# pytorch/audio

Measured on AMD Instinct MI355X. Metric: audio-sec/sec MelSpectrogram (b=256, 16kHz, n_fft=400, n_mels=80), higher is better.
Workload: dtype f32; 1 GPU; MelSpectrogram n_fft=400 hop=160 n_mels=80, batch=256 x 10 s @16 kHz fp32 per GPU (BASELINE configs[1]); per_gpu_batch=256

## Files before the change

audio_amd/csrc/melspec400.h:

```cpp
#pragma once
#include <cstdint>
#include <cstring>
#include <type_traits>
#include "hd.h"
#include "stft_generic.h"

namespace aamd {
namespace m400 {

constexpr int kN = 400;
constexpr int kPad = 200;
constexpr int kFramesPerWave = 6;
#ifndef AAMD_M400_WAVES
#define AAMD_M400_WAVES 12
#define AAMD_M400_MINWAVES 3
#endif
constexpr int kWavesPerBlock = AAMD_M400_WAVES;
constexpr int kTOff[20] = {0, 260, 520, 652, 784, 916, 1444, 1576, 128, 388,
                           2104, 2232, 2364, 1708, 1840, 1048, 1180, 1312, 1972, 2492};
constexpr int kTBufDwords = 2492 + 128;
constexpr int kTRow = 44;
constexpr int kTPair = 20 * kTRow;
constexpr int kLdsDwordsPerWave = 3 * kTPair;
constexpr int kPK = 208;
// ... 485 lines not shown
  const float m = sqrt(m2);
  if (power == 1.0f) return m;
  return pow(m, power);
}

AAMD_HD void phase_b2_spec(const LaneConst& c, const float (&zr)[20], const float (&zi)[20],
                           const float (&xr)[10], const float (&xi)[10], float power, int phase, float* lds) {
  if (!c.active) return;
  float* Ra = lds + phase + kSpecBins * 2 * c.p + c.col;
  float* Rb = Ra + kSpecBins;
#pragma unroll
  for (int u = 0; u < 10; ++u) {
    const float cr = xr[9 - u], ci = xi[9 - u];
    const float ar = zr[u] + cr, ai = zi[u] - ci;
    const float br = zr[u] - cr, bi = zi[u] + ci;
    Ra[20 * u] = spec_pow(ar * ar + ai * ai, power);
    Rb[20 * u] = spec_pow(br * br + bi * bi, power);
  }
  if (c.col == 0) {
    const float ar = zr[10] + zr[10], bi = zi[10] + zi[10];
    Ra[200] = spec_pow(ar * ar, power);
    Rb[200] = spec_pow(bi * bi, power);
  }
}

AAMD_HD void phase_b2_spec_complex(const LaneConst& c, const float (&zr)[20], const float (&zi)[20],
                                   const float (&xr)[10], const float (&xi)[10], int half, int phase, float* lds) {
  if (!c.active) return;
  const int fa = 2 * c.p - 3 * half, fb = fa + 1;
  const bool wa = fa >= 0 && fa < 3, wb = fb >= 0 && fb < 3;
  float* Ra = lds + phase + 2 * kSpecBins * fa + 2 * c.col;
  float* Rb = lds + phase + 2 * kSpecBins * fb + 2 * c.col;
#pragma unroll
  for (int u = 0; u < 10; ++u) {
    const float cr = xr[9 - u], ci = xi[9 - u];
    if (wa) { Ra[40 * u] = zr[u] + cr; Ra[40 * u + 1] = zi[u] - ci; }
    if (wb) { Rb[40 * u] = zi[u] + ci; Rb[40 * u + 1] = cr - zr[u]; }
  }
  if (c.col == 0) {
    if (wa) { Ra[400] = zr[10] + zr[10]; Ra[401] = 0.0f; }
    if (wb) { Rb[400] = zi[10] + zi[10]; Rb[401] = 0.0f; }
  }
}

AAMD_HD void store_spec(int lane, const float* lds, float* out, int64_t a0, int n_floats) {
  const int phase = (int)(a0 & 3);
  float* base = out + (a0 - phase);
  const int n_pieces = (phase + n_floats + 3) >> 2;
  for (int j = lane; j < n_pieces; j += 64) {
    const int i0 = 4 * j;
    if (i0 >= phase && i0 + 4 <= phase + n_floats) {
      *reinterpret_cast<F4*>(base + i0) = *reinterpret_cast<const F4*>(lds + i0);
    } else {
      for (int e = 0; e < 4; ++e)
        if (i0 + e >= phase && i0 + e < phase + n_floats) base[i0 + e] = lds[i0 + e];
    }
  }
}

#ifndef AAMD_M400_SPEC_FULL
#define AAMD_M400_SPEC_FULL 1
#endif
AAMD_HD void store_spec_full(int lane, const float* lds, float* out, int64_t a0) {
  constexpr int kN = kFramesPerWave * kSpecBins;
  const int phase = (int)(a0 & 3);
  float* base = out + (a0 - phase);
  const int n_pieces = (phase + kN + 3) >> 2;
  F4 v[5];
#pragma unroll
  for (int u = 0; u < 5; ++u) {
    const int j = lane + 64 * u;
    if (u < 4 || j < n_pieces) v[u] = *reinterpret_cast<const F4*>(lds + 4 * j);
  }
#pragma unroll
  for (int u = 0; u < 5; ++u) {
    const int j = lane + 64 * u, i0 = 4 * j;
    const bool full = i0 >= phase && i0 + 4 <= phase + kN;
    if ((u < 4 || j < n_pieces) && full) *reinterpret_cast<F4*>(base + i0) = v[u];
  }
  if (lane == 0 && phase != 0) {
    const float e[4] = {v[0].x, v[0].y, v[0].z, v[0].w};
#pragma unroll
    for (int k = 1; k < 4; ++k)
      if (k >= phase) base[k] = e[k];
  }
  const int jl = n_pieces - 1, il = 4 * jl;
  if (lane + 256 == jl && il + 4 > phase + kN) {
    const float e[4] = {v[4].x, v[4].y, v[4].z, v[4].w};
#pragma unroll
    for (int k = 0; k < 3; ++k)
      if (il + k < phase + kN) base[il + k] = e[k];
  }
}

AAMD_HD float fast_log10(float x) {
#if defined(__HIP_DEVICE_COMPILE__)
  return __log2f(x) * 0.30102999566398120f;
#else
  return log10(x);
#endif
}
AAMD_HD float epi_plog(float x) {
  const float kE = 2.718281828459045f;
#if defined(__HIP_DEVICE_COMPILE__)
  const float lg = __log2f(x) * 0.69314718055994531f;
#else
  const float lg = log(x);
#endif
  const float t = x > kE ? lg : x;
  return t <= kE ? t / kE : t;
}
AAMD_HD float epi_db(float x, const Epi400& e) {
  return e.multiplier * fast_log10(fmax(x, e.amin)) - e.db_sub;
}

AAMD_HD void phase_b2_pad(int lane, float* lds) {
  constexpr int kTail = kPK - 201;
  if (lane < 3 * kTail) {
    const int p = lane / kTail, j = lane - p * kTail;
    *reinterpret_cast<F2*>(lds + kPPair * p + 2 * (201 + j)) = F2{0.0f, 0.0f};
  }
}

template <int NC>
AAMD_HD void mel_chunks(const float* wt, const float* P, float& sa, float& sb) {
  F4 w[NC], q0[NC], q1[NC];
#pragma unroll
  for (int k = 0; k < NC; ++k) {
    w[k] = *reinterpret_cast<const F4*>(wt + 4 * k);
    q0[k] = *reinterpret_cast<const F4*>(P + 8 * k);
    q1[k] = *reinterpret_cast<const F4*>(P + 8 * k + 4);
  }
#pragma unroll
  for (int k = 0; k < NC; ++k) {
    sa += w[k].x * q0[k].x;
    sb += w[k].x * q0[k].y;
    sa += w[k].y * q0[k].z;
    sb += w[k].y * q0[k].w;
    sa += w[k].z * q1[k].x;
    sb += w[k].z * q1[k].y;
    sa += w[k].w * q1[k].z;
    sb += w[k].w * q1[k].w;
  }
}

template <int NR>
struct MelRegs {
  int nc[NR];
  int pm[NR];
  AAMD_HD int poff(int r) const { return pm[r] & 0xffff; }
  AAMD_HD int mel(int r) const { return pm[r] >> 16; }
};

template <int NR>
AAMD_HD void mel_regs_load(const LaneConst& c, const MelTab& mt, MelRegs<NR>& h) {
#pragma unroll
  for (int r = 0; r < NR; ++r) {
    const bool on = r < mt.n_rounds;
    const int row = r * kMelSlots + c.pi;
#if defined(__HIP_DEVICE_COMPILE__)
    h.nc[r] = on ? __builtin_amdgcn_readfirstlane(mt.rc[r]) : 0;
#else
    h.nc[r] = on ? mt.rc[r] : 0;
#endif
    const int poff = on ? 2 * mt.lo2[row] : 0;
    const int mel = on ? mt.row_mel[row] : -1;
    h.pm[r] = (int)(((unsigned)mel << 16) | (unsigned)poff);
  }
}

AAMD_HD constexpr int sig_chunks(int sig, int r) { return (sig >> (4 * r)) & 15; }
constexpr int kSigHtk80 = 0x4221, kSigSlaney80 = 0x4211;

template <int NR = kMelMaxRounds, int SIG = 0, bool FENCED = false>
AAMD_HD void phase_c(const LaneConst& c, const MelTab& mt, const float* lds,
                     float (&acc_a)[NR], float (&acc_b)[NR], const MelRegs<NR>* h = nullptr) {
  const float* Pp = lds + kPPair * c.p;
  const float* wt0 = mt.w + c.pi * mt.ws;
#pragma unroll
  for (int r = 0; r < NR; ++r) {
    float sa = 0.0f, sb = 0.0f;
#if defined(__HIP_DEVICE_COMPILE__)
    if (FENCED && SIG != 0 && r > 0 && (r & 1) == 0) __builtin_amdgcn_sched_barrier(0);
#endif
    if (SIG != 0 || r < mt.n_rounds) {
      const float* wt = wt0 + r * kMelSlots * mt.ws;
      const float* P = Pp + (h ? h->poff(r) : 2 * mt.lo2[r * kMelSlots + c.pi]);
      const int nc = SIG != 0 ? sig_chunks(SIG, r) : (h ? h->nc[r] : mt.rc[r]);
      switch (nc) {
        case 1: mel_chunks<1>(wt, P, sa, sb); break;
        case 2: mel_chunks<2>(wt, P, sa, sb); break;
        case 3: mel_chunks<3>(wt, P, sa, sb); break;
        case 4: mel_chunks<4>(wt, P, sa, sb); break;
        default:
          for (int k = 0; k < nc; ++k) mel_chunks<1>(wt + 4 * k, P + 8 * k, sa, sb);
      }
    }
    acc_a[r] = sa;
    acc_b[r] = sb;
  }
}

template <int OFF>
AAMD_HD void store_f32_saddr(float v, char* base, unsigned voff) {
#if defined(__HIP_DEVICE_COMPILE__)
  asm volatile("global_store_dword %0, %1, %2 offset:%3" : : "v"(voff), "v"(v), "s"(base), "i"(OFF) : "memory");
#else
  *reinterpret_cast<float*>(base + (size_t)voff + OFF) = v;
#endif
}

template <int NR = kMelMaxRounds, int SIG = 0>
AAMD_HD void store_direct(const LaneConst& c, const MelTab& mt, const float (&acc_a)[NR],
                          const float (&acc_b)[NR], float* out_row, int64_t t0, int n_frames,
                          const MelRegs<NR>* h = nullptr) {
  const int left = (int)(n_frames - t0);
  const bool va = c.active && 2 * c.p < left, vb = c.active && 2 * c.p + 1 < left;
  float* out_tile = out_row + t0 * (int64_t)mt.n_mels;
  const unsigned oa = 2u * (unsigned)c.p * (unsigned)mt.n_mels;
  if (SIG != 0) {
    constexpr unsigned nm = kMelSlots * NR;
    char* const ob = reinterpret_cast<char*>(out_row + t0 * (int64_t)nm);
    unsigned bo[NR];
#pragma unroll
    for (int r = 0; r < NR; ++r) bo[r] = 4u * (2u * (unsigned)c.p * nm + (unsigned)h->mel(r));
    if (left >= kFramesPerWave) {
      if (c.active) {
#pragma unroll
        for (int r = 0; r < NR; ++r) store_f32_saddr<0>(acc_a[r], ob, bo[r]);
#pragma unroll
        for (int r = 0; r < NR; ++r) store_f32_saddr<4 * (int)nm>(acc_b[r], ob, bo[r]);
      }
      return;
    }
    if (va) {
#pragma unroll
      for (int r = 0; r < NR; ++r) store_f32_saddr<0>(acc_a[r], ob, bo[r]);
    }
    if (vb) {
#pragma unroll
      for (int r = 0; r < NR; ++r) store_f32_saddr<4 * (int)nm>(acc_b[r], ob, bo[r]);
    }
    return;
  }
#pragma unroll
  for (int r = 0; r < NR; ++r) {
    if (r < mt.n_rounds) {
      const int m = h ? h->mel(r) : mt.row_mel[r * kMelSlots + c.pi];
      if (m >= 0) {
        if (va) out_tile[oa + (unsigned)m] = acc_a[r];
        if (vb) out_tile[oa + (unsigned)mt.n_mels + (unsigned)m] = acc_b[r];
      }
    }
  }
}

template <int NR = kMelMaxRounds>
AAMD_HD void store_stage(const LaneConst& c, const MelTab& mt, const float (&acc_a)[NR],
                         const float (&acc_b)[NR], float* lds, const MelRegs<NR>* h = nullptr) {
  if (!c.active) return;
  float* oa = lds + 2 * c.p * mt.n_mels;
#pragma unroll
  for (int r = 0; r < NR; ++r) {
    if (r < mt.n_rounds) {
      const int m = h ? h->mel(r) : mt.row_mel[r * kMelSlots + c.pi];
      if (m >= 0) {
        oa[m] = acc_a[r];
        oa[mt.n_mels + m] = acc_b[r];
      }
    }
  }
}

AAMD_HD void store_wide(int lane, const MelTab& mt, const float* lds, float* out_row, int64_t t0,
                        int n_frames) {
  const int64_t left = n_frames - t0;
  const int n_valid = left < kFramesPerWave ? (int)left : kFramesPerWave;
  const int pieces = n_valid * mt.n_mels / 4;
  float* dst = out_row + t0 * (int64_t)mt.n_mels;
  for (int j = lane; j < pieces; j += 64)
    *reinterpret_cast<F4*>(dst + 4 * j) = *reinterpret_cast<const F4*>(lds + 4 * j);
}

#if defined(__HIPCC__)
__device__ __forceinline__ float vmax_raw(float x, float y) {
  float r;
  asm("v_max_f32 %0, %1, %2" : "=v"(r) : "v"(x), "v"(y));
  return r;
}
__device__ __forceinline__ float vmin_raw(float x, float y) {
  float r;
  asm("v_min_f32 %0, %1, %2" : "=v"(r) : "v"(x), "v"(y));
  return r;
}
__device__ __forceinline__ float vmax3_raw(float x, float y, float z) {
  float r;
  asm("v_max3_f32 %0, %1, %2, %3" : "=v"(r) : "v"(x), "v"(y), "v"(z));
  return r;
}
__device__ __forceinline__ float vmin3_raw(float x, float y, float z) {
  float r;
  asm("v_min3_f32 %0, %1, %2, %3" : "=v"(r) : "v"(x), "v"(y), "v"(z));
  return r;
}
__device__ __forceinline__ void wave_lds_fence() {
  asm volatile("" ::: "memory");
}

__device__ __forceinline__ void exchange_partner(float (&qr)[10], float (&qi)[10], unsigned long long self_mask) {
  unsigned long long saved;
  asm volatile(
      "s_mov_b64 %[sv], exec\n\t"
      "s_andn2_b64 exec, exec, %[m]\n\t"
      "s_nop 4\n\t"
      "v_mov_b32_dpp %0, %0 quad_perm:[1,0,3,2] row_mask:0xf bank_mask:0xf\n\t"
      "v_mov_b32_dpp %1, %1 quad_perm:[1,0,3,2] row_mask:0xf bank_mask:0xf\n\t"
      "v_mov_b32_dpp %2, %2 quad_perm:[1,0,3,2] row_mask:0xf bank_mask:0xf\n\t"
      "v_mov_b32_dpp %3, %3 quad_perm:[1,0,3,2] row_mask:0xf bank_mask:0xf\n\t"
      "v_mov_b32_dpp %4, %4 quad_perm:[1,0,3,2] row_mask:0xf bank_mask:0xf\n\t"
      "v_mov_b32_dpp %5, %5 quad_perm:[1,0,3,2] row_mask:0xf bank_mask:0xf\n\t"
      "v_mov_b32_dpp %6, %6 quad_perm:[1,0,3,2] row_mask:0xf bank_mask:0xf\n\t"
      "v_mov_b32_dpp %7, %7 quad_perm:[1,0,3,2] row_mask:0xf bank_mask:0xf\n\t"
      "v_mov_b32_dpp %8, %8 quad_perm:[1,0,3,2] row_mask:0xf bank_mask:0xf\n\t"
      "v_mov_b32_dpp %9, %9 quad_perm:[1,0,3,2] row_mask:0xf bank_mask:0xf\n\t"
      "v_mov_b32_dpp %10, %10 quad_perm:[1,0,3,2] row_mask:0xf bank_mask:0xf\n\t"
      "v_mov_b32_dpp %11, %11 quad_perm:[1,0,3,2] row_mask:0xf bank_mask:0xf\n\t"
      "v_mov_b32_dpp %12, %12 quad_perm:[1,0,3,2] row_mask:0xf bank_mask:0xf\n\t"
      "v_mov_b32_dpp %13, %13 quad_perm:[1,0,3,2] row_mask:0xf bank_mask:0xf\n\t"
      "v_mov_b32_dpp %14, %14 quad_perm:[1,0,3,2] row_mask:0xf bank_mask:0xf\n\t"
      "v_mov_b32_dpp %15, %15 quad_perm:[1,0,3,2] row_mask:0xf bank_mask:0xf\n\t"
      "v_mov_b32_dpp %16, %16 quad_perm:[1,0,3,2] row_mask:0xf bank_mask:0xf\n\t"
      "v_mov_b32_dpp %17, %17 quad_perm:[1,0,3,2] row_mask:0xf bank_mask:0xf\n\t"
      "v_mov_b32_dpp %18, %18 quad_perm:[1,0,3,2] row_mask:0xf bank_mask:0xf\n\t"
      "v_mov_b32_dpp %19, %19 quad_perm:[1,0,3,2] row_mask:0xf bank_mask:0xf\n\t"
      "s_mov_b64 exec, %[sv]"
      : "+v"(qr[0]), "+v"(qr[1]), "+v"(qr[2]), "+v"(qr[3]), "+v"(qr[4]), "+v"(qr[5]), "+v"(qr[6]), "+v"(qr[7]),
        "+v"(qr[8]), "+v"(qr[9]), "+v"(qi[0]), "+v"(qi[1]), "+v"(qi[2]), "+v"(qi[3]), "+v"(qi[4]), "+v"(qi[5]),
        "+v"(qi[6]), "+v"(qi[7]), "+v"(qi[8]), "+v"(qi[9]), [sv] "=&s"(saved)
      : [m] "s"(self_mask));
}

__device__ __forceinline__ void glds16(const void* gsrc, unsigned lds_dst) {
  asm volatile("s_mov_b32 m0, %1\n\ts_nop 0\n\tglobal_load_lds_dwordx4 %0, off" : : "v"(gsrc), "s"(lds_dst) : "memory", "m0");
}

#ifndef AAMD_M400_DMA_SADDR
#define AAMD_M400_DMA_SADDR 1
#endif
__device__ __forceinline__ void glds16s(const void* sbase, unsigned voff_bytes, unsigned lds_dst) {
  asm volatile("s_mov_b32 m0, %2\n\ts_nop 0\n\tglobal_load_lds_dwordx4 %0, %1" : : "v"(voff_bytes), "s"(sbase), "s"(lds_dst) : "memory", "m0");
}
__device__ __forceinline__ void stage_wait() { asm volatile("s_waitcnt vmcnt(0)" ::: "memory"); }

struct TileInfo {
  int64_t row;
  int t0;
  bool staged;
  unsigned tin;
  int64_t in_off;
  int64_t out_off;
};

__device__ __forceinline__ void atomic_max_f32(float* addr, float v) {
  if (v >= 0.0f) atomicMax(reinterpret_cast<int*>(addr), __float_as_int(v));
  else atomicMin(reinterpret_cast<unsigned int*>(addr), __float_as_uint(v));
}

template <int LAB, int EPI, int H = 8, typename TIn = float, int NR = kMelMaxRounds, int SIG = 0>
__global__ void __launch_bounds__(64 * kWavesPerBlock, AAMD_M400_MINWAVES)
melspec400_kernel(const TIn* __restrict__ wav, const float* __restrict__ window,
                  const float* __restrict__ tw400, MelBandsDev mb, float* __restrict__ out,
                  int64_t rows, int64_t length, int64_t row_stride, int n_frames, float scale,
                  int tiles_per_row, int64_t n_tiles, int tiles_per_block, int in_aligned,
                  int out_wide, Epi400 epi) {
  extern __shared__ __attribute__((aligned(16))) float smem400[];
  unsigned fix_base = 0, fix_cnt = 0;
#if defined(AAMD_LAB) && defined(AAMD_MFCC_FIXUP_RETURNS)
  if (EPI == EPI400_MFCC && epi.fixup != 0) return;
#endif
  if (EPI == EPI400_MFCC && epi.fixup != 0) {
    int* const cnt = reinterpret_cast<int*>(smem400);
    if (threadIdx.x == 0) *cnt = 0;
    __syncthreads();
    const unsigned nt = (unsigned)n_tiles, nbk = gridDim.x, b = blockIdx.x;
    const unsigned n_cand = b < nt ? (nt - b + nbk - 1u) / nbk : 0u;
    fix_base = b * (nt / nbk) + (b < nt % nbk ? b : nt % nbk);
    for (unsigned k0 = 0; k0 < n_cand; k0 += blockDim.x) {
      const unsigned k = k0 + threadIdx.x;
      bool hit = false;
      unsigned t = 0;
      if (k < n_cand) {
        t = b + k * nbk;
        const unsigned row = t / (unsigned)tiles_per_row;
        hit = epi.tile_min[t] < epi.group_max[row / epi.rows_per_group] - epi.top_db;
      }
      const unsigned long long m = __ballot(hit);
      int slot = 0;
      if ((threadIdx.x & 63) == 0 && m)
        slot = __hip_atomic_fetch_add(cnt, __popcll(m), __ATOMIC_RELAXED, __HIP_MEMORY_SCOPE_WORKGROUP);
      slot = __builtin_amdgcn_readfirstlane(slot);
      if (hit) epi.fix_list[fix_base + slot + __popcll(m & ((1ull << (threadIdx.x & 63)) - 1ull))] = (int)t;
    }
    __syncthreads();
    fix_cnt = (unsigned)__builtin_amdgcn_readfirstlane(*cnt);
    if (fix_cnt == 0) return;
    if (threadIdx.x == 0) atomicAdd(epi.fix_count, (int)fix_cnt);
    __syncthreads();
  }
  if (EPI == EPI400_MFCC && epi.fixup == 0 && epi.fix_count != nullptr && !(LAB & (1048576 | 8388608)) && blockIdx.x == 0 &&
      threadIdx.x == 0)
    *epi.fix_count = 0;
  const int elab = (LAB & 524288) ? epi.lab : 0;
  const int lane = threadIdx.x & 63;
  const int wave = __builtin_amdgcn_readfirstlane(threadIdx.x >> 6);
#ifdef AAMD_M400_PRIO
  {
    const int pr = AAMD_M400_PRIO == 1 ? (wave >> 2) : AAMD_M400_PRIO == 2 ? 2 - (wave >> 2) : (wave >> 2) == 0 ? 1 : 0;
    if (pr == 1) __builtin_amdgcn_s_setprio(1);
    else if (pr == 2) __builtin_amdgcn_s_setprio(2);
  }
#endif
  long long lab_t0 = 0;
  if (LAB & 1024) lab_t0 = wall_clock64();
  if ((LAB & 1048576) && lane == 0) {
    long long* rec = reinterpret_cast<long long*>(epi.fix_count);
    const int w = blockIdx.x * kWavesPerBlock + wave;
    rec[4 * w] = (long long)clock64();
    rec[4 * w + 1] = wall_clock64();
  }
  using HC = Hop<H>;
  constexpr int kHop = HC::hop;
  float* lds = smem400 + wave * HC::lds_dwords;
  const unsigned s_addr = (unsigned)(uintptr_t)(lds + kSOff);

  float* const_tab = smem400 + kWavesPerBlock * HC::lds_dwords;
  const_tab_build(threadIdx.x, blockDim.x, window, tw400, scale, const_tab);
  MelTab mt{};
  const int tab_dwords = (EPI != EPI400_SPEC) ? mel_tab_dwords(mb.n_mels, mb.max_width) : 0;
  int* queue = reinterpret_cast<int*>(const_tab + kConstDwords + tab_dwords);
  constexpr bool kIoWave = (LAB & 16777216) != 0;
  constexpr int kNio = kIoWave ? ((LAB & 67108864) ? 2 : 1) : 0;
  if (threadIdx.x == 0) *queue = kWavesPerBlock - kNio;
  float* frag_lds = const_tab + kConstDwords + tab_dwords + 4;
  constexpr bool kFragLds = (H != 10);
  if (EPI == EPI400_MFCC && (epi.frag_in_lds != 0) != kFragLds) __builtin_trap();
  if (EPI == EPI400_MFCC && kFragLds)
    for (int i = threadIdx.x; i < kMfccFragFloats; i += blockDim.x) frag_lds[i] = epi.dct_frag[i];
  if (EPI != EPI400_SPEC && mb.table400 != nullptr) {
    float* dst = const_tab + kConstDwords;
    for (int i = threadIdx.x; i < tab_dwords; i += blockDim.x) dst[i] = mb.table400[i];
    mel_tab_layout(mb, dst, mt);
    __syncthreads();
  } else {
    if (EPI != EPI400_SPEC) mel_tab_rounds(threadIdx.x, blockDim.x, mb, const_tab + kConstDwords, mt);
    __syncthreads();
    if (EPI != EPI400_SPEC) mel_tab_fill(threadIdx.x, blockDim.x, mb, const_tab + kConstDwords, mt);
    __syncthreads();
  }

  long long lab_t1 = 0;
  if (LAB & 1024) lab_t1 = wall_clock64();
  LaneConst c;
  lane_init(lane, const_tab, c);
  constexpr bool kWinRegs = (EPI != EPI400_MFCC || H != 10) && (((LAB & 8192) != 0) || !(LAB & 262144));
  float winr[20], twr[40];
  if (kWinRegs) {
#pragma unroll
    for (int q = 0; q < 20; ++q) winr[q] = c.win[q];
  }
#ifndef AAMD_M400_TWREG
#define AAMD_M400_TWREG 3
#endif
#ifndef AAMD_M400_TWREG_DB
#define AAMD_M400_TWREG_DB 1
#endif
#ifndef AAMD_M400_TWREG_MFCC
#define AAMD_M400_TWREG_MFCC 2
#endif
  constexpr bool kPlain = H == 8 && std::is_same<TIn, float>::value && LAB == 0;
  constexpr int kTwRegBatches = (LAB & 16384) ? 4
                                : (SIG != 0 && EPI == EPI400_MEL) ? AAMD_M400_TWREG
                                : !kPlain ? 0
                                : EPI == EPI400_SPEC ? 2
                                : (EPI == EPI400_MEL && SIG == 0) ? (NR <= 4 ? 1 : 3)
                                : (EPI == EPI400_MFCC && NR <= 4) ? AAMD_M400_TWREG_MFCC
                                : (EPI == EPI400_MEL_DB && NR <= 4) ? AAMD_M400_TWREG_DB : 0;
  if (kTwRegBatches > 0) {
#pragma unroll
    for (int q = 0; q < 10 * kTwRegBatches; ++q) twr[q] = c.tw[q];
  }
  constexpr bool kHoist = NR <= 4;
  MelRegs<NR> mregs;
  const MelRegs<NR>* mh = nullptr;
  if (EPI != EPI400_SPEC && kHoist) {
    mel_regs_load<NR>(c, mt, mregs);
    mh = &mregs;
  }
  if (SIG != 0) {
    static_assert(SIG == 0 || NR == 4, "filterbank signatures are 4 rounds of 20 mels");
    const int sig_rt = mregs.nc[0] | (mregs.nc[1 % NR] << 4) | (mregs.nc[2 % NR] << 8) | (mregs.nc[3 % NR] << 12);
    if (mt.n_rounds != NR || mt.n_mels != kMelSlots * NR || sig_rt != SIG) __builtin_trap();
  }
  if (EPI == EPI400_MFCC && (mt.n_rounds != NR || mt.n_mels != kMelSlots * NR)) __builtin_trap();
  float nrm_mean[NR], nrm_inv[NR];
  if (EPI == EPI400_MEL_NORM) {
#pragma unroll
    for (int r = 0; r < NR; ++r) {
      const int m = r < mt.n_rounds ? mt.row_mel[r * kMelSlots + c.pi] : -1;
      nrm_mean[r] = m >= 0 ? epi.mean[m] : 0.0f;
      nrm_inv[r] = m >= 0 ? epi.invstd[m] : 0.0f;
    }
  }
  const unsigned long long self_mask = __ballot((c.col == 0) || (c.col == 10));
  using SG = Stage<H, TIn>;
  static_assert(SG::ok, "no staging layout for this hop / input type");
  int spiece[SG::ndma];
#pragma unroll
  for (int k = 0; k < SG::ndma; ++k) spiece[k] = SG::spp * stage_src_piece<H, TIn>(64 * k + lane);

  const int nb = gridDim.x;
  int lb = blockIdx.x;
  if ((nb & 7) == 0) lb = (blockIdx.x & 7) * (nb >> 3) + (blockIdx.x >> 3);
  unsigned blk_first = (unsigned)lb * (unsigned)tiles_per_block;
  unsigned blk_count = 0;
  if (blk_first < (unsigned)n_tiles) {
    blk_count = (unsigned)n_tiles - blk_first;
    if (blk_count > (unsigned)tiles_per_block) blk_count = (unsigned)tiles_per_block;
  }
  if (EPI == EPI400_MFCC && epi.fixup != 0) {
    blk_first = 0;
    blk_count = fix_cnt;
  }
  const unsigned queue_addr = (unsigned)(uintptr_t)queue;
  auto claim = [&]() {
    int v = 0;
    if (lane == 0)
      asm volatile("ds_add_rtn_u32 %0, %1, %2\n\ts_waitcnt lgkmcnt(0)" : "=v"(v) : "v"(queue_addr), "v"(1) : "memory");
    return (unsigned)__builtin_amdgcn_readfirstlane(v);
  };
#if AAMD_M400_POOLS
#define AAMD_M400_POOLED (AAMD_M400_POOLS && (LAB == 0) && epi.pool != nullptr && !(EPI == EPI400_MFCC && epi.fixup != 0))
  if (AAMD_M400_POOLED && blk_count > (unsigned)(tiles_per_block - epi.pool_p)) blk_count = (unsigned)(tiles_per_block - epi.pool_p);
  unsigned pool_ticket = 0;
  auto pool_request = [&]() {
    int lbo = (int)(blk_first / (unsigned)tiles_per_block);
    asm volatile("" : "+s"(lbo));
    unsigned* const ctr = epi.pool + (lbo % pool_count(nb)) * kPoolStride;
    if (lane == 0) pool_ticket = __hip_atomic_fetch_add(ctr, 1u, __ATOMIC_RELAXED, __HIP_MEMORY_SCOPE_AGENT);
  };
  auto pool_take = [&]() {
    int lbo = (int)(blk_first / (unsigned)tiles_per_block);
    asm volatile("" : "+s"(lbo));
    const int np = pool_count(nb), pid = lbo % np, mem = pool_members(nb, np, pid);
    for (;;) {
      const unsigned v = (unsigned)__builtin_amdgcn_readfirstlane((int)pool_ticket);
      if (v + 1u == (unsigned)(mem * (epi.pool_p + kWavesPerBlock)) && lane == 0)
        __hip_atomic_store(epi.pool + pid * kPoolStride, 0u, __ATOMIC_RELAXED, __HIP_MEMORY_SCOPE_AGENT);
      bool exhausted;
      const unsigned t = pool_tile(np, epi.pool_p, tiles_per_block, (unsigned)n_tiles, pid, mem, v, exhausted);
      if (t != kNoTile) return t - blk_first;
      if (exhausted) return 0x80000000u;
      pool_request();
    }
  };
  constexpr unsigned kBadIdx = 0x80000000u, kPendIdx = 0x80000001u;
#define AAMD_M400_IDX_OK(I) ((((I) ^ 0x80000000u)) > 1u)
#define AAMD_M400_LOCAL(I) ((I) < blk_count ? (I) : kBadIdx)
#else
#define AAMD_M400_IDX_OK(I) ((I) < blk_count)
#define AAMD_M400_LOCAL(I) (I)
#endif
  constexpr unsigned kLabChunk = 8;
  unsigned* gq = reinterpret_cast<unsigned*>(epi.group_max);
  int g_pending = 0;
  unsigned g_base = 0, g_pos = 0;
  auto g_request = [&]() {
    if (lane == 0) g_pending = (int)__hip_atomic_fetch_add(gq, 1u, __ATOMIC_RELAXED, __HIP_MEMORY_SCOPE_AGENT);
  };
  if (LAB & 131072) {
    blk_count = (unsigned)n_tiles;
    g_request();
    g_base = (unsigned)__builtin_amdgcn_readfirstlane(g_pending) * kLabChunk;
    g_request();
  }
  auto g_next = [&]() {
    if (++g_pos < kLabChunk) return g_base + g_pos;
    g_base = (unsigned)__builtin_amdgcn_readfirstlane(g_pending) * kLabChunk;
    g_pos = 0;
    g_request();
    return g_base;
  };

  static_assert(kFramesPerWave * kHop >= kPad, "tile 1 starts inside the clip");
  unsigned tin_hi = 0;
  if (in_aligned && length >= kN - kPad) {
    int64_t last = (length - (kN - kPad)) / kHop - (kFramesPerWave - 1);
    if (last > (int64_t)n_frames - kFramesPerWave) last = (int64_t)n_frames - kFramesPerWave;
    if (last >= kFramesPerWave) tin_hi = (unsigned)(last / kFramesPerWave);
  }
  const int64_t out_row_elems =
      EPI == EPI400_SPEC   ? (int64_t)n_frames * (epi.power > 0.0f ? kSpecBins : 2 * kSpecBins)
      : EPI == EPI400_MFCC ? (int64_t)n_frames * epi.n_mfcc
                           : (EPI == EPI400_MEL_NORM ? epi.out_frames : (int64_t)n_frames) * (int64_t)mb.n_mels;
  auto tile_fill = [&](TileInfo& ti, unsigned idx) {
    ti.t0 = (int)ti.tin * kFramesPerWave;
    ti.staged = AAMD_M400_IDX_OK(idx) && ti.tin - 1u < tin_hi;
  };
  auto tile_info = [&](unsigned idx) {
    TileInfo ti;
    unsigned t = ((LAB & 131072) ? 0u : blk_first) + idx;
    if (EPI == EPI400_MFCC && epi.fixup != 0)
      t = idx < blk_count ? (unsigned)__hip_atomic_load(epi.fix_list + fix_base + idx, __ATOMIC_RELAXED, __HIP_MEMORY_SCOPE_AGENT) : 0u;
    const unsigned row = t / (unsigned)tiles_per_row;
    ti.row = row;
    ti.tin = t - row * (unsigned)tiles_per_row;
    ti.in_off = (ti.row / InTraits<TIn>::chans) * row_stride;
    ti.out_off = ti.row * out_row_elems;
    tile_fill(ti, idx);
    return ti;
  };
  constexpr bool kCarry = !(LAB & (131072 | 16777216)) && !AAMD_M400_POOLS && EPI != EPI400_MFCC && InTraits<TIn>::chans == 1;
  constexpr unsigned kCarryMinTiles = 16;
  auto tile_next = [&](const TileInfo& from, unsigned from_idx, unsigned idx) {
    if (!kCarry || (unsigned)tiles_per_row < kCarryMinTiles) return tile_info(idx);
    TileInfo ti = from;
    if (!(AAMD_M400_IDX_OK(idx))) {
      ti.staged = false;
      return ti;
    }
    ti.tin = from.tin + (idx - from_idx);
    while (ti.tin >= (unsigned)tiles_per_row) {
      ti.tin -= (unsigned)tiles_per_row;
      ti.row += 1;
      ti.in_off += row_stride;
      ti.out_off += out_row_elems;
    }
    tile_fill(ti, idx);
    return ti;
  };
  auto stage_issue = [&](const TileInfo& ti) {
    const TIn* src = wav + ti.in_off + ((int64_t)ti.t0 * kHop - kPad);
    if (LAB & 32) src = wav + 6 * kHop;
#pragma unroll
    for (int k = 0; k < SG::ndma; ++k)
      if (!(LAB & 64) || k == 0) {
#if AAMD_M400_DMA_SADDR
        glds16s(src, (unsigned)spiece[k] * (unsigned)sizeof(TIn), s_addr + 1024 * k);
#else
        glds16(src + spiece[k], s_addr + 1024 * k);
#endif
      }
  };

  float wmax = -INFINITY;
  int64_t wgroup = -1, wrow = -1;
  constexpr bool kDb = (EPI == EPI400_MEL_DB) || (EPI == EPI400_MFCC);
  const bool fix = (EPI == EPI400_MFCC) && epi.fixup != 0;
  auto flush_max = [&]() {
    if (kDb && !fix && epi.group_max != nullptr && wgroup >= 0) {
      float m = wmax;
#pragma unroll
      for (int off = 32; off > 0; off >>= 1) m = fmaxf(m, __shfl_xor(m, off, 64));
      if (lane == 0) atomic_max_f32(epi.group_max + wgroup, m);
    }
    wmax = -INFINITY;
  };

  if (kIoWave && wave >= kWavesPerBlock - kNio) {
    constexpr unsigned D = 8;
    constexpr bool kFetchOnly = (LAB & 134217728) != 0;
    if (!(LAB & 33554432)) {
      const unsigned n_mine = (blk_count + (unsigned)kNio - 1u - (unsigned)(wave - (kWavesPerBlock - kNio))) / (unsigned)kNio;
      for (unsigned i = 0; i < n_mine + D; ++i) {
        const unsigned t = i * (unsigned)kNio + (unsigned)(wave - (kWavesPerBlock - kNio));
        if (i < n_mine) {
          const TileInfo ti = tile_info(AAMD_M400_LOCAL(t));
          const unsigned dst = (unsigned)(uintptr_t)(smem400 + (t % (unsigned)kWavesPerBlock) * HC::lds_dwords + kSOff);
          if (ti.staged) {
            const TIn* src = wav + ti.in_off + ((int64_t)ti.t0 * kHop - kPad);
#pragma unroll
            for (int k = 0; k < SG::ndma; ++k) glds16(src + spiece[k], dst + 1024 * k);
          }
        }
        if (i >= D) {
          if (kFetchOnly) {
            asm volatile("s_waitcnt vmcnt(40)" ::: "memory");
          } else {
            asm volatile("s_waitcnt vmcnt(56)" ::: "memory");
            const unsigned told = t - D * (unsigned)kNio;
            const TileInfo to = tile_info(AAMD_M400_LOCAL(told));
            const float* stg = smem400 + (told % (unsigned)kWavesPerBlock) * HC::lds_dwords;
            store_wide(lane, mt, stg, out + to.row * (int64_t)n_frames * (int64_t)mb.n_mels, to.t0, n_frames);
          }
        }
      }
    }
    blk_count = 0;
  }
  unsigned cur_idx = (LAB & 131072) ? g_base : (unsigned)wave;
#if AAMD_M400_POOLS
  if (cur_idx >= blk_count) cur_idx = kBadIdx;
  if (AAMD_M400_POOLED && cur_idx == kBadIdx) {
    pool_request();
    cur_idx = pool_take();
  }
#endif
  TileInfo cur = tile_info(cur_idx);
  if (LAB & 128) {
    const int k = (wave + 6 * lb) % 3;
    for (int i = 0; i < k; ++i) __builtin_amdgcn_s_sleep(112);
  }
  if (LAB & 2048) {
    const int k = 4 * (wave & 3) + (wave >> 2) % 3;
    for (int i = 0; i < (k % 12); ++i) __builtin_amdgcn_s_sleep(17);
  }
  if (LAB & 4096) {
    const int k = 4 * ((wave >> 2) % 3) + (wave & 3);
    for (int i = 0; i < k; ++i) __builtin_amdgcn_s_sleep(17);
  }
  float Xn[HC::nx];
  auto gload = [&](const TileInfo& ti) {
    const TIn* src = wav + ti.in_off + ((int64_t)ti.t0 * kHop - kPad) + (HC::pair_stride * c.p + c.pi);
#pragma unroll
    for (int q = 0; q < HC::nx; ++q) Xn[q] = InTraits<TIn>::get(src + 20 * q, (int)(ti.row % InTraits<TIn>::chans));
  };
  if (LAB & 32768) {
#pragma unroll
    for (int q = 0; q < HC::nx; ++q) Xn[q] = 0.0f;
    if (cur.staged) gload(cur);
  } else if (cur.staged && !(LAB & 8) && !fix) {
    stage_issue(cur);
  }

  long long ph_acc[6] = {0, 0, 0, 0, 0, 0}, ph_t = 0;
  int ph_tiles = 0;
#define AAMD_M400_STAMP(K)                                  \
  if (LAB & 8388608) {                                      \
    const long long now_ = (long long)clock64();            \
    ph_acc[K] += now_ - ph_t;                               \
    ph_t = now_;                                            \
  }
  using mfcc_f32x4 = __attribute__((ext_vector_type(4))) float;
  mfcc_f32x4 cf[kMfccMT];
  const int mfcc_elab = (LAB & 524288) ? epi.lab : 0;
  auto mfcc_finish = [&](int64_t row, int64_t t0) {
#pragma unroll
    for (int t = 0; t < kMfccMT; ++t)
#pragma unroll
      for (int i = 0; i < 4; ++i) {
        cf[t][i] += __int_as_float(__builtin_amdgcn_mov_dpp(__float_as_int(cf[t][i]), 0x128, 0xf, 0xf, true));
        asm volatile("" : "+v"(cf[t][i]));
      }
    const int64_t left64 = n_frames - t0;
    const int left = left64 < kFramesPerWave ? (int)left64 : kFramesPerWave;
    if (!(LAB & 2) && !(mfcc_elab & 8) && (lane & 15) < left) {
      float* otile = out + (row * (int64_t)n_frames + t0) * (int64_t)epi.n_mfcc;
      const unsigned ooff = (unsigned)(lane & 15) * (unsigned)epi.n_mfcc + 4u * (unsigned)(lane >> 4);
#pragma unroll
      for (int t = 0; t < kMfccMT; ++t) {
        const int k0 = 16 * t + 4 * (lane >> 4);
        if (k0 < epi.n_mfcc) *reinterpret_cast<F4*>(otile + (ooff + 16u * (unsigned)t)) = F4{cf[t][0], cf[t][1], cf[t][2], cf[t][3]};
      }
    }
  };
  while (AAMD_M400_IDX_OK(cur_idx)) {
    if (LAB & 8388608) { ph_t = (long long)clock64(); ++ph_tiles; }
#if AAMD_M400_POOLS
    unsigned nxt_idx = (LAB & 131072) ? g_next() : claim();
    if (nxt_idx >= blk_count) nxt_idx = AAMD_M400_POOLED ? kPendIdx : kBadIdx;
#else
    const unsigned nxt_idx = (LAB & 131072) ? g_next() : claim();
#endif
    TileInfo nxt = tile_next(cur, cur_idx, nxt_idx);
    float fix_cut = -INFINITY;
    if (fix) {
      fix_cut = epi.group_max[cur.row / epi.rows_per_group] - epi.top_db;
      if (cur.staged) stage_issue(cur);
    }

    float X[HC::nx];
    if ((LAB & 32768) && cur.staged) {
#pragma unroll
      for (int q = 0; q < HC::nx; ++q) X[q] = Xn[q];
    } else if (cur.staged) {
      if (!(LAB & 1)) stage_wait();
      if (LAB & 256) {
#pragma unroll
        for (int q = 0; q < HC::nx; ++q) X[q] = (float)(q + lane) * scale;
      } else {
        gather_lds<H, TIn>(c, reinterpret_cast<const TIn*>(lds + kSOff), X, (int)(cur.row % InTraits<TIn>::chans));
      }
    } else {
      gather_global<H, TIn>(c, wav + cur.in_off, length, cur.t0, n_frames, X,
                            (int)(cur.row % InTraits<TIn>::chans));
    }
#if AAMD_M400_POOLS
    if (nxt_idx == kPendIdx) pool_request();
#endif
    phase_a<H, kWinRegs, kTwRegBatches>(c, X, lds, winr, twr);
    if ((LAB & 32768) && nxt.staged) gload(nxt);
    wave_lds_fence();
    AAMD_M400_STAMP(0)
    float vr[20], vi[20], zr[20], zi[20], qr[10], qi[10];
    phase_b1_load(c, lds, vr, vi);
    if (!(LAB & 32768)) {
      asm volatile("s_waitcnt lgkmcnt(0)" ::: "memory");
      AAMD_M400_STAMP(1)
#if AAMD_M400_POOLS
      if (nxt_idx == kPendIdx) {
        nxt_idx = pool_take();
        nxt = tile_info(nxt_idx);
      }
#endif
      if (nxt.staged && !(LAB & 8) && !fix) stage_issue(nxt);
    }
    if (LAB & 16) { wave_lds_fence(); cur = nxt; cur_idx = nxt_idx; continue; }
    dft20(vr, vi, zr, zi);
    phase_b2_send(c, zr, zi, qr, qi);
    exchange_partner(qr, qi, self_mask);
    wave_lds_fence();
    AAMD_M400_STAMP(2)
    if (EPI == EPI400_SPEC) {
      const int64_t left = n_frames - cur.t0;
      const int n_valid = left < kFramesPerWave ? (int)left : kFramesPerWave;
      if (epi.power > 0.0f) {
        const int64_t a0 = cur.out_off + (int64_t)cur.t0 * kSpecBins;
        phase_b2_spec(c, zr, zi, qr, qi, epi.power, (int)(a0 & 3), lds);
        wave_lds_fence();
        if (!(LAB & 2)) {
          if (AAMD_M400_SPEC_FULL && n_valid == kFramesPerWave) store_spec_full(lane, lds, out, a0);
          else store_spec(lane, lds, out, a0, n_valid * kSpecBins);
        }
        wave_lds_fence();
      } else {
#pragma unroll
        for (int half = 0; half < 2; ++half) {
          const int64_t a0 = cur.out_off + (int64_t)(cur.t0 + 3 * half) * (2 * kSpecBins);
          const int nv = n_valid - 3 * half < 3 ? n_valid - 3 * half : 3;
          phase_b2_spec_complex(c, zr, zi, qr, qi, half, (int)(a0 & 3), lds);
          wave_lds_fence();
          if (!(LAB & 2) && nv > 0) store_spec(lane, lds, out, a0, nv * 2 * kSpecBins);
          wave_lds_fence();
        }
      }
      cur = nxt;
      cur_idx = nxt_idx;
      continue;
    }
    phase_b2(c, zr, zi, qr, qi, lds);
    phase_b2_pad(lane, lds);
    wave_lds_fence();
    AAMD_M400_STAMP(3)
    float acc_a[NR], acc_b[NR];
    if (LAB & 4) { wave_lds_fence(); cur = nxt; cur_idx = nxt_idx; continue; }
    phase_c<NR, SIG, EPI == EPI400_MFCC>(c, mt, lds, acc_a, acc_b, mh);
    if (LAB & 8388608) { asm volatile("" : "+v"(acc_a[0]), "+v"(acc_b[NR - 1])); }
    AAMD_M400_STAMP(4)
    if (kDb) {
      if (cur.row != wrow) {
        wrow = cur.row;
        const int64_t g = cur.row / epi.rows_per_group;
        if (g != wgroup) {
          flush_max();
          wgroup = g;
        }
      }
      const bool va_ok = cur.t0 + 2 * c.p < n_frames, vb_ok = cur.t0 + 2 * c.p + 1 < n_frames;
      float tmin = INFINITY;
      if (EPI == EPI400_MFCC) {
        const float db_c1 = epi.multiplier * 0.30102999566398120f;
#pragma unroll
        for (int r = 0; r < NR; ++r) {
          acc_a[r] = __builtin_fmaf(__log2f(vmax_raw(acc_a[r], epi.amin)), db_c1, -epi.db_sub);
          acc_b[r] = __builtin_fmaf(__log2f(vmax_raw(acc_b[r], epi.amin)), db_c1, -epi.db_sub);
        }
        if (cur.t0 + kFramesPerWave <= n_frames) {
#pragma unroll
          for (int r = 0; r < NR; ++r) {
            wmax = vmax3_raw(wmax, acc_a[r], acc_b[r]);
            tmin = vmin3_raw(tmin, acc_a[r], acc_b[r]);
          }
        } else {
#pragma unroll
          for (int r = 0; r < NR; ++r) {
            wmax = fmaxf(wmax, fmaxf(va_ok ? acc_a[r] : -INFINITY, vb_ok ? acc_b[r] : -INFINITY));
            tmin = fminf(tmin, fminf(va_ok ? acc_a[r] : INFINITY, vb_ok ? acc_b[r] : INFINITY));
          }
        }
        if (fix) {
#pragma unroll
          for (int r = 0; r < NR; ++r) {
            acc_a[r] = vmax_raw(acc_a[r], fix_cut);
            acc_b[r] = vmax_raw(acc_b[r], fix_cut);
          }
        }
      } else {
        const bool interior = cur.t0 + kFramesPerWave <= n_frames;
#pragma unroll
        for (int r = 0; r < NR; ++r) {
          if (r < mt.n_rounds) {
            acc_a[r] = epi.multiplier * fast_log10(vmax_raw(acc_a[r], epi.amin)) - epi.db_sub;
            acc_b[r] = epi.multiplier * fast_log10(vmax_raw(acc_b[r], epi.amin)) - epi.db_sub;
            if (interior) wmax = vmax3_raw(wmax, acc_a[r], acc_b[r]);
            else wmax = fmaxf(wmax, fmaxf(va_ok ? acc_a[r] : -INFINITY, vb_ok ? acc_b[r] : -INFINITY));
          }
        }
      }
      if (EPI == EPI400_MFCC && !fix && !(elab & 4)) {
        asm volatile(
            "s_nop 1\n\t"
            "v_min_f32_dpp %0, %0, %0 row_shr:1 row_mask:0xf bank_mask:0xf\n\ts_nop 1\n\t"
            "v_min_f32_dpp %0, %0, %0 row_shr:2 row_mask:0xf bank_mask:0xf\n\ts_nop 1\n\t"
            "v_min_f32_dpp %0, %0, %0 row_shr:4 row_mask:0xf bank_mask:0xf\n\ts_nop 1\n\t"
            "v_min_f32_dpp %0, %0, %0 row_shr:8 row_mask:0xf bank_mask:0xf\n\ts_nop 1\n\t"
            "v_min_f32_dpp %0, %0, %0 row_bcast:15 row_mask:0xa bank_mask:0xf\n\ts_nop 1\n\t"
            "v_min_f32_dpp %0, %0, %0 row_bcast:31 row_mask:0xc bank_mask:0xf"
            : "+v"(tmin));
        if (lane == 63) epi.tile_min[blk_first + cur_idx] = tmin;
      }
    }
    if (EPI == EPI400_MFCC) {
      using f32x4 = __attribute__((ext_vector_type(4))) float;
      using h8 = __attribute__((ext_vector_type(8))) _Float16;
      using h4 = __attribute__((ext_vector_type(4))) _Float16;
      using u32x4 = __attribute__((ext_vector_type(4))) uint32_t;
      using u32x2 = __attribute__((ext_vector_type(2))) uint32_t;
      wave_lds_fence();
      {
        uint16_t* hs = reinterpret_cast<uint16_t*>(lds);
        uint16_t* ls = hs + kMfccPlaneHalves;
#pragma unroll
        for (int r = 0; r < NR; ++r) {
          const int m = mh ? mh->mel(r) : mt.row_mel[r * kMelSlots + c.pi];
          const float va = acc_a[r] * kMfccYScale, vb = acc_b[r] * kMfccYScale;
          const _Float16 ha = (_Float16)va, hb = (_Float16)vb;
          const _Float16 la = (_Float16)(va - (float)ha), lb = (_Float16)(vb - (float)hb);
          hs[2 * c.p * kMfccMels + m] = __builtin_bit_cast(uint16_t, ha);
          ls[2 * c.p * kMfccMels + m] = __builtin_bit_cast(uint16_t, la);
          hs[(2 * c.p + 1) * kMfccMels + m] = __builtin_bit_cast(uint16_t, hb);
          ls[(2 * c.p + 1) * kMfccMels + m] = __builtin_bit_cast(uint16_t, lb);
        }
      }
      wave_lds_fence();
#pragma unroll
      for (int t = 0; t < kMfccMT; ++t) cf[t] = f32x4{0.0f, 0.0f, 0.0f, 0.0f};
      auto product = [&](const u32x4* __restrict__ ftab) {
        const uint16_t* hs = reinterpret_cast<const uint16_t*>(lds);
        u32x4 a0[kMfccMT][2];
        auto frag_load = [&](int sidx) {
#pragma unroll
          for (int t = 0; t < kMfccMT; ++t)
#pragma unroll
            for (int hl = 0; hl < 2; ++hl) {
              a0[t][hl] = u32x4{0x3c003c00u, 0x3c003c00u, 0x3c003c00u, 0x3c003c00u};
              if (!(elab & 1)) a0[t][hl] = ftab[mfcc_frag_piece(t, sidx, hl, lane)];
            }
        };
#pragma unroll
        for (int sidx = 0; sidx < 2; ++sidx) {
          const h8 bb = __builtin_bit_cast(h8, *reinterpret_cast<const u32x4*>(hs + mfcc_b_index(lane, sidx)));
          frag_load(sidx);
#pragma unroll
          for (int t = 0; t < kMfccMT; ++t)
            cf[t] = __builtin_amdgcn_mfma_f32_16x16x32_f16(__builtin_bit_cast(h8, a0[t][1]), bb, cf[t], 0, 0, 0);
#pragma unroll
          for (int t = 0; t < kMfccMT; ++t)
            cf[t] = __builtin_amdgcn_mfma_f32_16x16x32_f16(__builtin_bit_cast(h8, a0[t][0]), bb, cf[t], 0, 0, 0);
        }
        {
          frag_load(2);
          const h4 bb = __builtin_bit_cast(h4, *reinterpret_cast<const u32x2*>(hs + mfcc_b_index(lane, 2)));
#define AAMD_A4(T, HL) __builtin_bit_cast(h4, u32x2{a0[T][HL][0], a0[T][HL][1]})
#pragma unroll
          for (int t = 0; t < kMfccMT; ++t) cf[t] = __builtin_amdgcn_mfma_f32_16x16x16f16(AAMD_A4(t, 1), bb, cf[t], 0, 0, 0);
#pragma unroll
          for (int t = 0; t < kMfccMT; ++t) cf[t] = __builtin_amdgcn_mfma_f32_16x16x16f16(AAMD_A4(t, 0), bb, cf[t], 0, 0, 0);
#undef AAMD_A4
        }
      };
      if (!(elab & 2)) {
        if (kFragLds) product(reinterpret_cast<const u32x4*>(frag_lds));
        else product(reinterpret_cast<const u32x4*>(epi.dct_frag));
      }
      if (!(elab & 2)) mfcc_finish(cur.row, cur.t0);
      wave_lds_fence();
      cur = nxt;
      cur_idx = nxt_idx;
      continue;
    }
    if (EPI == EPI400_MEL_NORM) {
#pragma unroll
      for (int r = 0; r < NR; ++r) {
        if (r < mt.n_rounds) {
          acc_a[r] = (epi_plog(acc_a[r] * epi.gain) - nrm_mean[r]) * nrm_inv[r];
          acc_b[r] = (epi_plog(acc_b[r] * epi.gain) - nrm_mean[r]) * nrm_inv[r];
        }
      }
    }
    float* out_row = out + cur.out_off;
    if (LAB & 4194304) out_row = out + (int64_t)(wave + kWavesPerBlock * (blockIdx.x & 63)) * 6 * mb.n_mels - cur.t0 * (int64_t)mb.n_mels;
    if (out_wide) {
      wave_lds_fence();
      store_stage<NR>(c, mt, acc_a, acc_b, lds, mh);
      wave_lds_fence();
      if (!(LAB & 2)) store_wide(lane, mt, lds, out_row, cur.t0, n_frames);
    } else {
      if (!(LAB & 2)) store_direct<NR, SIG>(c, mt, acc_a, acc_b, out_row, cur.t0, n_frames, mh);
    }
    wave_lds_fence();
    AAMD_M400_STAMP(5)
    cur = nxt;
    cur_idx = nxt_idx;
  }
#undef AAMD_M400_STAMP
  if ((LAB & 8388608) && lane == 0) {
    long long* rec = reinterpret_cast<long long*>(epi.fix_count) + 4 * 12 * 256 + 8 * (blockIdx.x * kWavesPerBlock + wave);
#pragma unroll
    for (int k = 0; k < 6; ++k) rec[k] = ph_acc[k];
    rec[6] = ph_tiles;
  }
  if (kDb && !fix && epi.group_max != nullptr) {
    float m = wmax;
#pragma unroll
    for (int off = 32; off > 0; off >>= 1) m = fmaxf(m, __shfl_xor(m, off, 64));
    if (lane == 0) {
      reinterpret_cast<int*>(lds)[0] = (int)wgroup;
      lds[1] = m;
    }
    __syncthreads();
    if (threadIdx.x == 0) {
      int g_run = -1;
      float m_run = -INFINITY;
      for (int w = 0; w < kWavesPerBlock; ++w) {
        const int gw = reinterpret_cast<const int*>(smem400 + w * HC::lds_dwords)[0];
        const float mw = smem400[w * HC::lds_dwords + 1];
        if (gw != g_run) {
          if (g_run >= 0) atomic_max_f32(epi.group_max + g_run, m_run);
          g_run = gw;
          m_run = mw;
        } else {
          m_run = fmaxf(m_run, mw);
        }
      }
      if (g_run >= 0) atomic_max_f32(epi.group_max + g_run, m_run);
    }
  }
  if ((LAB & 1048576) && lane == 0) {
    long long* rec = reinterpret_cast<long long*>(epi.fix_count);
    const int w = blockIdx.x * kWavesPerBlock + wave;
    rec[4 * w + 2] = (long long)clock64();
    rec[4 * w + 3] = wall_clock64();
  }
  if ((LAB & 1024) && lane == 0) {
    long long* rec = reinterpret_cast<long long*>(const_cast<float*>(tw400) + 1024);
    const int w = blockIdx.x * kWavesPerBlock + wave;
    rec[3 * w] = lab_t0;
    rec[3 * w + 1] = lab_t1;
    rec[3 * w + 2] = wall_clock64();
  }
}
#endif

}
}
```

Measured before the change: 38.29 million audio-sec/sec.

## Batch prologue global loads before LDS stores to overlap table setup latency

Rewrites the kernel prologue so the constant twiddle/window table, the mel table copy and the MFCC DCT fragment are first loaded into registers all at once, then written to LDS. Table copies use 16-byte vector loads when aligned. For the mel signature path, the per-round mel register loads are also issued in one batch before use. The aim is to cut serialized global-load latency in the per-block setup, at the cost of more registers in the prologue. It also extends the lab timing instrumentation with an extra timestamp.

```diff
diff --git a/audio_amd/csrc/melspec400.h b/audio_amd/csrc/melspec400.h
--- a/audio_amd/csrc/melspec400.h
+++ b/audio_amd/csrc/melspec400.h
@@ -661,19 +661,43 @@
   AAMD_HD int mel(int r) const { return pm[r] >> 16; }
 };
 
-template <int NR>
+template <int NR, bool BATCH = false>
 AAMD_HD void mel_regs_load(const LaneConst& c, const MelTab& mt, MelRegs<NR>& h) {
+  if (!BATCH) {
+#pragma unroll
+    for (int r = 0; r < NR; ++r) {
+      const bool on = r < mt.n_rounds;
+      const int row = r * kMelSlots + c.pi;
+#if defined(__HIP_DEVICE_COMPILE__)
+      h.nc[r] = on ? __builtin_amdgcn_readfirstlane(mt.rc[r]) : 0;
+#else
+      h.nc[r] = on ? mt.rc[r] : 0;
+#endif
+      const int poff = on ? 2 * mt.lo2[row] : 0;
+      const int mel = on ? mt.row_mel[row] : -1;
+      h.pm[r] = (int)(((unsigned)mel << 16) | (unsigned)poff);
+    }
+    return;
+  }
+  int rc[NR], lo2[NR], rm[NR];
+#pragma unroll
+  for (int r = 0; r < NR; ++r) {
+    const int rr = r < mt.n_rounds ? r : 0;
+    const int row = rr * kMelSlots + c.pi;
+    rc[r] = mt.rc[rr];
+    lo2[r] = mt.lo2[row];
+    rm[r] = mt.row_mel[row];
+  }
 #pragma unroll
   for (int r = 0; r < NR; ++r) {
     const bool on = r < mt.n_rounds;
-    const int row = r * kMelSlots + c.pi;
 #if defined(__HIP_DEVICE_COMPILE__)
-    h.nc[r] = on ? __builtin_amdgcn_readfirstlane(mt.rc[r]) : 0;
+    h.nc[r] = on ? __builtin_amdgcn_readfirstlane(rc[r]) : 0;
 #else
-    h.nc[r] = on ? mt.rc[r] : 0;
-#endif
-    const int poff = on ? 2 * mt.lo2[row] : 0;
-    const int mel = on ? mt.row_mel[row] : -1;
+    h.nc[r] = on ? rc[r] : 0;
+#endif
+    const int poff = on ? 2 * lo2[r] : 0;
+    const int mel = on ? rm[r] : -1;
     h.pm[r] = (int)(((unsigned)mel << 16) | (unsigned)poff);
   }
 }
@@ -942,8 +966,20 @@
   float* lds = smem400 + wave * HC::lds_dwords;
   const unsigned s_addr = (unsigned)(uintptr_t)(lds + kSOff);
 
+  constexpr int kThreads = 64 * kWavesPerBlock;
+  const int tid = threadIdx.x;
   float* const_tab = smem400 + kWavesPerBlock * HC::lds_dwords;
-  const_tab_build(threadIdx.x, blockDim.x, window, tw400, scale, const_tab);
+  constexpr int kCtIters = (20 * 20 + kThreads - 1) / kThreads;
+  float ct_re[kCtIters], ct_im[kCtIters], ct_w[kCtIters];
+#pragma unroll
+  for (int k = 0; k < kCtIters; ++k) {
+    const int i = tid + k * kThreads < 20 * 20 ? tid + k * kThreads : 20 * 20 - 1;
+    const int b = i / 20, s = i - 20 * b;
+    const int idx = (b * s) % kN;
+    ct_re[k] = tw400[2 * idx];
+    ct_im[k] = tw400[2 * idx + 1];
+    ct_w[k] = window[b + 20 * s];
+  }
   MelTab mt{};
   const int tab_dwords = (EPI != EPI400_SPEC) ? mel_tab_dwords(mb.n_mels, mb.max_width) : 0;
   int* queue = reinterpret_cast<int*>(const_tab + kConstDwords + tab_dwords);
@@ -953,12 +989,52 @@
   float* frag_lds = const_tab + kConstDwords + tab_dwords + 4;
   constexpr bool kFragLds = (H != 10);
   if (EPI == EPI400_MFCC && (epi.frag_in_lds != 0) != kFragLds) __builtin_trap();
-  if (EPI == EPI400_MFCC && kFragLds)
-    for (int i = threadIdx.x; i < kMfccFragFloats; i += blockDim.x) frag_lds[i] = epi.dct_frag[i];
-  if (EPI != EPI400_SPEC && mb.table400 != nullptr) {
-    float* dst = const_tab + kConstDwords;
-    for (int i = threadIdx.x; i < tab_dwords; i += blockDim.x) dst[i] = mb.table400[i];
-    mel_tab_layout(mb, dst, mt);
+  const bool tab_copy = EPI != EPI400_SPEC && mb.table400 != nullptr;
+  float* const tab_dst = const_tab + kConstDwords;
+  const int tab_pieces = (tab_copy && (reinterpret_cast<uintptr_t>(mb.table400) & 15) == 0) ? tab_dwords >> 2 : 0;
+  F4 tab_p0 = F4{0.0f, 0.0f, 0.0f, 0.0f};
+  if (tab_pieces > 0) tab_p0 = reinterpret_cast<const F4*>(mb.table400)[tid < tab_pieces ? tid : tab_pieces - 1];
+  constexpr int kFragPieces = kMfccFragFloats / 4;
+  constexpr int kFragIters = (EPI == EPI400_MFCC && kFragLds) ? (kFragPieces + kThreads - 1) / kThreads : 0;
+  F4 frag_p[kFragIters > 0 ? kFragIters : 1];
+#pragma unroll
+  for (int k = 0; k < kFragIters; ++k) {
+    const int i = tid + k * kThreads;
+    frag_p[k] = reinterpret_cast<const F4*>(epi.dct_frag)[i < kFragPieces ? i : kFragPieces - 1];
+  }
+#pragma unroll
+  for (int k = 0; k < kCtIters; ++k) {
+    const int i = tid + k * kThreads;
+    if (i < 20 * 20) {
+      const int b = i / 20, s = i - 20 * b;
+      const_tab[kTwRow * b + 2 * s] = ct_re[k];
+      const_tab[kTwRow * b + 2 * s + 1] = ct_im[k];
+      const_tab[20 * kTwRow + i] = ct_w[k] * (0.5f * scale);
+    }
+  }
+  if (tid < tab_pieces) reinterpret_cast<F4*>(tab_dst)[tid] = tab_p0;
+#pragma unroll
+  for (int k = 0; k < kFragIters; ++k) {
+    const int i = tid + k * kThreads;
+    if (i < kFragPieces) reinterpret_cast<F4*>(frag_lds)[i] = frag_p[k];
+  }
+  if (tab_copy) {
+    for (int i = tid + kThreads; i < tab_pieces; i += kThreads)
+      reinterpret_cast<F4*>(tab_dst)[i] = reinterpret_cast<const F4*>(mb.table400)[i];
+    for (int i0 = 4 * tab_pieces + tid; i0 < tab_dwords; i0 += 4 * kThreads) {
+      float v[4];
+#pragma unroll
+      for (int k = 0; k < 4; ++k) {
+        const int i = i0 + k * kThreads;
+        v[k] = mb.table400[i < tab_dwords ? i : tab_dwords - 1];
+      }
+#pragma unroll
+      for (int k = 0; k < 4; ++k) {
+        const int i = i0 + k * kThreads;
+        if (i < tab_dwords) tab_dst[i] = v[k];
+      }
+    }
+    mel_tab_layout(mb, tab_dst, mt);
     __syncthreads();
   } else {
     if (EPI != EPI400_SPEC) mel_tab_rounds(threadIdx.x, blockDim.x, mb, const_tab + kConstDwords, mt);
@@ -967,7 +1043,7 @@
     __syncthreads();
   }
 
-  long long lab_t1 = 0;
+  long long lab_t1 = 0, lab_t2 = 0;
   if (LAB & 1024) lab_t1 = wall_clock64();
   LaneConst c;
   lane_init(lane, const_tab, c);
@@ -1002,7 +1078,7 @@
   MelRegs<NR> mregs;
   const MelRegs<NR>* mh = nullptr;
   if (EPI != EPI400_SPEC && kHoist) {
-    mel_regs_load<NR>(c, mt, mregs);
+    mel_regs_load<NR, SIG != 0 && EPI == EPI400_MEL>(c, mt, mregs);
     mh = &mregs;
   }
   if (SIG != 0) {
@@ -1306,6 +1382,10 @@
 #if AAMD_M400_POOLS
     if (nxt_idx == kPendIdx) pool_request();
 #endif
+    if ((LAB & 1024) && lab_t2 == 0) {
+      asm volatile("s_waitcnt vmcnt(0) lgkmcnt(0)" : "+v"(X[0]), "+v"(X[HC::nx - 1]) : : "memory");
+      lab_t2 = wall_clock64();
+    }
     phase_a<H, kWinRegs, kTwRegBatches>(c, X, lds, winr, twr);
     if ((LAB & 32768) && nxt.staged) gload(nxt);
     wave_lds_fence();
@@ -1561,14 +1641,15 @@
     rec[4 * w + 3] = wall_clock64();
   }
   if ((LAB & 1024) && lane == 0) {
-    long long* rec = reinterpret_cast<long long*>(const_cast<float*>(tw400) + 1024);
+    long long* rec = reinterpret_cast<long long*>(epi.fix_count);
     const int w = blockIdx.x * kWavesPerBlock + wave;
-    rec[3 * w] = lab_t0;
-    rec[3 * w + 1] = lab_t1;
-    rec[3 * w + 2] = wall_clock64();
-  }
-}
-#endif
-
-}
-}
+    rec[4 * w] = lab_t0;
+    rec[4 * w + 1] = lab_t1;
+    rec[4 * w + 2] = lab_t2;
+    rec[4 * w + 3] = wall_clock64();
+  }
+}
+#endif
+
+}
+}
```

Measured after the change: 38.42 million audio-sec/sec, median of 6. Within noise of the previous version (+0.3%).
